# brunohs1993/Nanokappa

Hardware: AMD Instinct MI355X
Metric: phonon-steps/sec (whole node) (higher is better)
Workload: dtype f64

## Files before the change

include/nanokappa_hip.h:

```cpp
#ifndef NANOKAPPA_HIP_H
#define NANOKAPPA_HIP_H
#include <stdint.h>

#ifdef __cplusplus
extern "C" {
#endif

typedef struct nk_ctx nk_ctx;

enum nk_status {
    NK_OK = 0,
    NK_ERR_HIP = -1,
    NK_ERR_ARG = -2,
    NK_ERR_CAPACITY = -3,
    NK_ERR_COMM = -4,
    NK_ERR_NODEVICE = -5
};

typedef struct {
    int32_t Q, J, NT;
    const double *omega;
    const double *group_vel;
    const double *T_grid;
    const double *lifetime;
// ... 103 lines not shown
    double place_gbps;
    double place_worst_gbps;
    int64_t box_store;
} nk_timing;

int nk_device_count(void);
int nk_mesh_crossings(int device, int64_t n_rays, const double *origins, const double *dirs, int64_t n_faces, const double *v0,
                      const double *e1, const double *e2, int skip_self, int32_t *counts);
int nk_create(nk_ctx **out, int device_id, uint64_t seed);
void nk_destroy(nk_ctx *ctx);
const char *nk_last_error(const nk_ctx *ctx);

int nk_set_material(nk_ctx *ctx, const nk_material *m);
int nk_set_mesh(nk_ctx *ctx, const nk_mesh *m);
int nk_set_subvolumes(nk_ctx *ctx, const nk_subvols *s, const double *T_sv_init );
int nk_set_reservoirs(nk_ctx *ctx, const nk_reservoirs *r);
int nk_set_rough(nk_ctx *ctx, const nk_rough *r);
int nk_set_params(nk_ctx *ctx, const nk_params *p);

int nk_reserve(nk_ctx *ctx, int64_t capacity);
int nk_upload_particles(nk_ctx *ctx, int64_t N, const double *x, const double *y, const double *z,
                        const int32_t *mode, const double *occ, const double *n_ts, const int32_t *facet,
                        const uint64_t *pid, uint64_t pid_offset);
int nk_init_boundaries(nk_ctx *ctx);
int nk_init_particles(nk_ctx *ctx, int64_t N, int64_t capacity, uint64_t pid_lo, const int32_t *unique_modes, int64_t n_unique,
                      const int64_t *sv_first);
int nk_tally_state(nk_ctx *ctx, double *E_raw, double *N_sv, double *flux_raw);
int nk_step(nk_ctx *ctx, int32_t nsteps, nk_tally *out);
int nk_download_particles(nk_ctx *ctx, int64_t capacity, double *x, double *y, double *z, int32_t *mode,
                          double *occ, double *n_ts, int32_t *facet, uint64_t *pid, int64_t *N_out);
int nk_get_subvol_temperature(nk_ctx *ctx, double *T_sv );
int nk_set_subvol_temperature(nk_ctx *ctx, const double *T_sv );
int nk_get_step(nk_ctx *ctx, int64_t *step);
int nk_get_timing(nk_ctx *ctx, nk_timing *t);

int nk_comm_unique_id(void *id128 );
int nk_comm_init(nk_ctx *ctx, const void *id128, int rank, int nranks);
typedef struct {
    int32_t rank, nranks;
    int32_t comm_rank, comm_nranks;
    int32_t device;
    int32_t selftest_ok;
    double selftest_sum;
    char pci_bus_id[32];
} nk_comm_report;
int nk_comm_info(nk_ctx *ctx, nk_comm_report *out);
int nk_comm_allreduce(nk_ctx *ctx, double *inout, int64_t n);

int nk_set_bands(nk_ctx *ctx, int32_t nbands, const int32_t *band_of_mode);
int nk_get_band_rows(nk_ctx *ctx, double *F, double *N, int64_t *steps, int32_t cap, int32_t *nrows);
int nk_tally_bands_state(nk_ctx *ctx, double *F, double *N);

typedef struct {
    double lo[3], h[3];
    int32_t n[3];
    int32_t every;
    int32_t flags;
    int64_t capacity;
} nk_field;
#define NK_FIELD_GLOBAL 1
#define NK_FIELD_TEST_SMALL_BOUND 2
int nk_set_field(nk_ctx *ctx, const nk_field *f);
int nk_get_field(nk_ctx *ctx, double *N, double *E, double *F, int64_t *samples, int64_t *clamped, int32_t reset);
int nk_tally_field_state(nk_ctx *ctx, int64_t *raw, int64_t *clamped);
typedef struct {
    int32_t n[3], every;
// ... 84 lines not shown
```

nanokappa_amd/csrc/nk_device.h:

```cpp
#pragma once
#include <hip/hip_runtime.h>
#include <stdint.h>

#define NK_WG 256
#ifndef NK_NREP
#define NK_NREP 8
#endif
#define NK_PLANE_DOUBLES 6
#define NK_FACE_DOUBLES 16
#define NK_LDS_FACES 256
#define NK_LDS_RESFACES 64
#define NK_TAU_ROWS 3
#define NK_MAX_SEGMENTS 16384
#define NK_EMIT_CHUNK 128
#define NK_LREC 128
#define NK_NEWBORN 0x80000000u
#define NK_LOST 0x40000000u

#define NK_TAG_REFLECT 0x00000u
#define NK_TAG_EMIT 0x10000u
#define NK_TAG_RESAMP 0x20000u
#define NK_TAG_DICE 0x30000u
#define NK_TAG_INIT 0x40000u

// ... 42 lines not shown
    const int32_t *m2s;
    const int32_t *s2m;
    const int32_t *seg_nl;
    int32_t tau_row0;
    double tau_g[NK_TAU_ROWS];
    double tau_ig[NK_TAU_ROWS - 1];
    double T0, invT0;
    double c_hk;
    const double *tau;
    const double *Tgrid;
    int32_t nE;
    const double *Tarr, *Earr;
    double Tfill_lo, Tfill_hi;
    double hbar, kb, QV;
    double active_modes;
    int32_t F, Fc, NP;
    const float *tree_boxes;
    double tree_bound;
    const int32_t *tree_tags;
    const double *facet_skip;
    const double *tree_faces;
    int32_t tree_base[8];
    int32_t tree_top, tree_leaves;
    int32_t tree_nfam, tree_lds_fam0, tree_lds_off;
    int32_t NG;
    const double *planes;
    const double *faces;
    const NkFacet *facets;
    double tol;
    double bbox[6];
    int32_t box;
    double box_k[6];
    uint64_t box_ids;
    double inv_dt;
    const double *face_verts;
    const int32_t *facet_face_off;
    const int32_t *facet_face_idx;
    const double *facet_face_cdf;
    int32_t nS;
    const double *simplex_pts;
    const double *simplex_cdf;
    int32_t S, sv_kind, sv_axis, sv_interp;
    const double *centers;
    const double *sv_volume;
    double sv_lo, sv_invL;
    double *T_sv;
    const double *rbf_inv;
    int32_t rbf_P, rbf_used[3];
    double rbf_shift[3], rbf_scale[3];
    int32_t R, res_gen;
    const int32_t *res_facet;
    const double *res_T;
    const int32_t *res_face_off;
    const double *res_face_cdf;
    const double *res_face_verts;
    int32_t res_nf;
    int32_t res_lds;
    const double *enter_prob;
    double *res_counter;
    const double *ep_p;
    double *rc_p;
    int64_t rc_len;
    const double *res_roulette;
    int32_t *nleave_prev;
    uint64_t *sp_inbox;
    int32_t *sp_inbox_n;
// ... 359 lines not shown
    NkHit h = {__builtin_inf(), 0x7fffffff, -1};
    {
#pragma clang fp contract(off)
        const double2 *P = reinterpret_cast<const double2 *>(planes);
        double tmin = __builtin_inf();
        int pmin = -1, ties = 0;
        double2 n0 = P[0], n1 = P[1];
        for (int pl = 0; pl < NP; ++pl) {
            const double2 p01 = n0, p23 = n1;
            if (pl + 1 < NP) { n0 = P[3 * pl + 3]; n1 = P[3 * pl + 4]; }
            const double num = x * p01.x + y * p01.y + z * p23.x + p23.y;
            const double den = vx * p01.x + vy * p01.y + vz * p23.x;
            if (!((num < 0.0 && den > 0.0) || (num > 0.0 && den < 0.0))) continue;
            const double t = -num / den;
            if (!(t >= tol) || isinf(t)) continue;
            if (t < tmin) { tmin = t; pmin = pl; ties = 0; }
            else if (t == tmin) ties = 1;
        }
        if (pmin < 0) { tc = h.t; fc = h.facet; return; }
        if (!ties) {
            const double cx = x + tmin * vx, cy = y + tmin * vy, cz = z + tmin * vz;
            const double pr = planes[NK_PLANE_DOUBLES * pmin + 4];
            nk_fb_faces(faces, __double2loint(pr), __double2hiint(pr), tol, tmin, cx, cy, cz, h);
            if (h.facet >= 0 || h.face != 0x7fffffff) { tc = h.t; fc = h.facet; return; }
        }
    }
    nk_fb_planes(planes, faces, 0, NP, tol, x, y, z, vx, vy, vz, h);
    tc = h.t;
    fc = h.facet;
}
struct NkBoxWalls {
    double lx, hx, ly, hy, lz, hz;
    uint32_t ids_lo, ids_hi;
    __device__ __forceinline__ void load(const NkDev &d) {
        lx = d.box_k[0]; hx = -d.box_k[1]; ly = d.box_k[2]; hy = -d.box_k[3]; lz = d.box_k[4]; hz = -d.box_k[5];
        ids_lo = (uint32_t)d.box_ids; ids_hi = (uint32_t)(d.box_ids >> 32);
        asm volatile("" : "+v"(lx), "+v"(hx), "+v"(ly), "+v"(hy), "+v"(lz), "+v"(hz), "+v"(ids_lo), "+v"(ids_hi));
    }
};
__device__ __forceinline__ bool nk_box_out(const NkBoxWalls &b, double x, double y, double z, double vx, double vy, double vz) {
    const bool ox = ((x > b.hx) & (vx > 0.0)) | ((x < b.lx) & (vx < 0.0));
    const bool oy = ((y > b.hy) & (vy > 0.0)) | ((y < b.ly) & (vy < 0.0));
    const bool oz = ((z > b.hz) & (vz > 0.0)) | ((z < b.lz) & (vz < 0.0));
    return ox | oy | oz;
}
__device__ __forceinline__ void nk_box_axis(double xa, double va, double lo, double hi, int wlo, uint64_t ids,
                                            double &nb, double &db, int &wb) {
#pragma clang fp contract(off)
    const bool fwd = va > 0.0;
    const double num = fwd ? xa - hi : lo - xa;
    const double den = fabs(va);
    const int w = wlo + (fwd ? 1 : 0);
    const double l = num * db, r = nb * den;
    const unsigned f0w = (unsigned)(ids >> (8 * w + 4)) & 15u, f0b = wb < 0 ? 16u : ((unsigned)(ids >> (8 * wb + 4)) & 15u);
    if ((num > 0.0) & (den > 0.0) & ((l > r) | ((l == r) & (f0w < f0b)))) { nb = num; db = den; wb = w; }
}
__device__ __forceinline__ void nk_box_first_hit(const NkBoxWalls &b, double inv_dt, double x, double y, double z, double vx, double vy,
                                                 double vz, double &nts, int &facet) {
    const uint64_t ids = ((uint64_t)b.ids_hi << 32) | b.ids_lo;
    double nb = -1.0, db = 1.0;
    int wb = -1;
    nk_box_axis(x, vx, b.lx, b.hx, 0, ids, nb, db, wb);
    nk_box_axis(y, vy, b.ly, b.hy, 2, ids, nb, db, wb);
    nk_box_axis(z, vz, b.lz, b.hz, 4, ids, nb, db, wb);
    nts = -(nb * nk_rcp(db)) * inv_dt;
    facet = wb < 0 ? -1 : (int)((ids >> (8 * wb)) & 15u);
}
__device__ __forceinline__ void nk_box_next_axis(double xa, double va, double lo, double hi, int wlo, uint64_t ids, double tol,
                                                 double &mb, double &db, int &wb) {
#pragma clang fp contract(off)
    const bool fwd = va > 0.0;
    const double num = fwd ? xa - hi : lo - xa;
    const double den = fabs(va), m = -num;
    const int w = wlo + (fwd ? 1 : 0);
    const double l = m * db, r = mb * den;
    const unsigned f0w = (unsigned)(ids >> (8 * w + 4)) & 15u, f0b = wb < 0 ? 16u : ((unsigned)(ids >> (8 * wb + 4)) & 15u);
    if ((num < 0.0) & (den > 0.0) & (m >= tol * den) & ((wb < 0) | (l < r) | ((l == r) & (f0w < f0b)))) { mb = m; db = den; wb = w; }
// ... 217 lines not shown
#endif
        const double r = r_diff * rlast;
        int flat;
        if (hi - lo <= 4) {
            const double a0 = lo + 0 < hi ? roul[lo + 0] : __builtin_inf(), a1 = lo + 1 < hi ? roul[lo + 1] : __builtin_inf(),
                         a2 = lo + 2 < hi ? roul[lo + 2] : __builtin_inf(), a3 = lo + 3 < hi ? roul[lo + 3] : __builtin_inf();
            flat = lo + (a0 < r ? 1 : 0) + (a1 < r ? 1 : 0) + (a2 < r ? 1 : 0) + (a3 < r ? 1 : 0);
            if (flat > hi) flat = hi;
        } else flat = lo + nk_ss_left(roul + lo, hi - lo, r);
        if (flat > d.M - 1) flat = d.M - 1;
        mode_out = flat;
        omega_out = d.modetab[flat].omega;
        E0_out = d.modetab[flat].E0;
        double invT;
        nk_interp_T<RBF>(d, tb, cx, cy, cz, invT);
        n_out = nk_be(omega_out * d.c_hk, E0_out, invT, d.invT0);
    }
}

struct NkBins {
    double *E, *flux, *resb;
    unsigned int *N, *nleave, *misc;
};

struct NkParticle {
    double x, y, z, occ, nts, omega, E0, vx, vy, vz;
    int mode, facet;
    int slot;
};

#define NK_EV_DONE 0
#define NK_EV_DEAD 1
#define NK_EV_MORE 2
template <bool ROUGH, bool RBF = true>
__device__ __forceinline__ int nk_event_pre(const NkDev &d, const NkFacet *facets, const NkSvTab &tb, const double *resT, NkBins &b,
                                            NkParticle &p, double &cts, uint32_t ev, uint64_t pid, uint32_t step) {
    const double dt = d.dt;
    int fi = p.facet < 0 ? d.Fc - 1 : p.facet;
    const NkFacet fc = facets[fi];
    if (fc.bc == 'T' || fc.bc == 'F') {
        int r = p.facet < 0 ? -1 : fc.res;
        if (r >= 0) {
            const double n0 = d.T_ref_local ? nk_be(p.omega * d.c_hk, p.E0, resT[2 * r + 1], d.invT0)
                                            : nk_occupation(d, d.T_ref, p.omega, p.E0);
            double e = d.hbar * p.omega * (p.occ - n0);
            const double evn = e * nk_rcp(p.vx * fc.nx + p.vy * fc.ny + p.vz * fc.nz);
            atomicAdd(&b.nleave[r], 1u);
            atomicAdd(&b.resb[4 * r + 0], -e);
            atomicAdd(&b.resb[4 * r + 1], evn * p.vx);
            atomicAdd(&b.resb[4 * r + 2], evn * p.vy);
            atomicAdd(&b.resb[4 * r + 3], evn * p.vz);
        }
        return NK_EV_DEAD;
    }
    double tcol = p.nts * dt;
    double cx = p.x + p.vx * tcol, cy = p.y + p.vy * tcol, cz = p.z + p.vz * tcol;
    cts += (cts == 0.0) ? fabs(p.nts + 1.0) : fabs(p.nts);
    if (fc.bc == 'P') {
        p.x = cx + fc.tx; p.y = cy + fc.ty; p.z = cz + fc.tz;
    } else if (ROUGH) {
        double r0, r1;
        nk_uniform2_dev(d.seed, pid, step, NK_TAG_REFLECT + ev, r0, r1);
        p.x = cx; p.y = cy; p.z = cz;
        int mo; double no, oo, eo;
        nk_reflect<RBF>(d, tb, fc.rough, p.mode, cx, cy, cz, p.occ, p.omega, p.E0, r0, r1, r1, mo, no, oo, eo);
        p.mode = mo; p.occ = no; p.omega = oo; p.E0 = eo;
        const NkMode *rec = d.modetab + mo;
        if (d.part) p.slot = d.m2s[mo];
        p.vx = rec->vx; p.vy = rec->vy; p.vz = rec->vz;
    }
    return NK_EV_MORE;
}
__device__ __forceinline__ int nk_event_post(const NkDev &d, NkParticle &p, double &cts, uint32_t &ev, double tc, int fcn) {
    const double dt = d.dt;
    p.nts = tc / dt;
    p.facet = fcn;
    if (++ev > 4096u) cts = 1.0;
    if (cts < 1.0) {
        const double rem = 1.0 - cts;
        if (rem > p.nts) return NK_EV_MORE;
        p.x += p.vx * dt * rem; p.y += p.vy * dt * rem; p.z += p.vz * dt * rem;
        p.nts -= rem;
    }
    return NK_EV_DONE;
}
// ... 32 lines not shown
```

nanokappa_amd/csrc/nk_engine.hip:

```cpp
#include <hip/hip_runtime.h>
#include <dlfcn.h>
#include <math.h>
#include <stdio.h>
#include <stdlib.h>
#include <string.h>
#include <algorithm>
#include <functional>
#include <queue>
#include <string>
#include <type_traits>
#include <chrono>
#include <time.h>
#include <vector>

#include <rccl/rccl.h>

#include "../../include/nanokappa_hip.h"
#include "nk_kernels.h"
#include "nk_field.h"
#include "nk_modes.h"
#include "nk_group.h"
#ifndef NK_PLAIN_IN_ENGINE
extern template __global__ void k_sweep<1, false, false, false, false, true, 1>(NkDev, uint32_t, int, int);
extern template __global__ void k_sweep<1, false, false, false, false, true, 2>(NkDev, uint32_t, int, int);
extern template __global__ void k_sweep<1, false, false, false, false, false, 1>(NkDev, uint32_t, int, int);
extern template __global__ void k_sweep<1, false, false, false, false, false, 2>(NkDev, uint32_t, int, int);
extern template __global__ void k_sweep<1, false, false, false, false, true, 1, true>(NkDev, uint32_t, int, int);
extern template __global__ void k_sweep<1, false, false, false, false, true, 2, true>(NkDev, uint32_t, int, int);
extern template __global__ void k_sweep<1, false, false, false, false, false, 1, true>(NkDev, uint32_t, int, int);
extern template __global__ void k_sweep<1, false, false, false, false, false, 2, true>(NkDev, uint32_t, int, int);
#endif

struct NkRccl {
    void *lib = nullptr;
    ncclResult_t (*GetUniqueId)(ncclUniqueId *) = nullptr;
    ncclResult_t (*CommInitRank)(ncclComm_t *, int, ncclUniqueId, int) = nullptr;
    ncclResult_t (*AllReduce)(const void *, void *, size_t, ncclDataType_t, ncclRedOp_t, ncclComm_t, hipStream_t) = nullptr;
    ncclResult_t (*CommDestroy)(ncclComm_t) = nullptr;
    ncclResult_t (*CommCount)(const ncclComm_t, int *) = nullptr;
    ncclResult_t (*CommUserRank)(const ncclComm_t, int *) = nullptr;
    ncclResult_t (*CommAbort)(ncclComm_t) = nullptr;
};

static thread_local std::string g_create_error;

struct nk_ctx {
    int device = 0;
    hipStream_t stream = nullptr;
    std::string err;
    NkDev d;
    std::vector<void *> allocs;
    std::vector<void *> pallocs;
    void *store_buf = nullptr;
    size_t store_pad = 0;
    bool store_pid = false;
    bool store_nts = true;
    bool mesh_box = false;
    bool box_forbidden = false;
    int32_t *anomalies = nullptr;
    bool have_material = false, have_mesh = false, have_sv = false, have_params = false;
    int64_t step = 0;
    bool pending_relax = false;
    int g_sweep = 0;
    std::vector<int32_t> h_seg_count;
    std::vector<hipEvent_t> evpool;
    int g_sweep_key = -1;
    size_t g_sweep_lds = 0;
    int layout_key = -1;
    std::vector<double> h_enter_prob;
    int64_t spec_M = 0;
    double *spec_v = nullptr, *spec_om = nullptr, *spec_dl = nullptr, *spec_svx = nullptr;
    int32_t *spec_rank = nullptr;
    double spec_vmax = 0.0;
    NkSpecMode *spec_modes = nullptr;
    int32_t *spec_in = nullptr, *spec_out = nullptr;
    unsigned long long *spec_count = nullptr;
    double *ks_kv = nullptr, *ks_mat = nullptr;
    double ks_tol[3] = {0, 0, 0};
    int64_t ks_Q = 0;
    int64_t spec_cap = 0;
    int64_t spec_last = 0;
    int rb_Fr = 0;
    double *rb_k2 = nullptr, *rb_nin = nullptr, *rb_eta = nullptr, *rb_sub = nullptr, *rb_spec = nullptr, *rb_roul = nullptr;
    uint8_t *rb_ts = nullptr;
    unsigned int *rb_map = nullptr;
    std::vector<int32_t> rb_facet;
    int64_t o2o_first = 0;
    bool stepped = false;
    int64_t emitted_for = -1;
    std::vector<double> h_vg;
// ... 703 lines not shown
            if (seen & (1 << w)) { ok = false; break; }
            seen |= 1 << w;
            const double wall = sgn ? -pn[3] : pn[3];
            if (!(fabs(wall - m->bbox[(sgn ? 3 : 0) + a]) <= 1e-9 * (1.0 + fabs(wall)))) { ok = false; break; }
            if (members[pl].size() != 2) { ok = false; break; }
            int fct0 = -1, face0 = 0x7fffffff;
            double area = 0.0;
            for (int f : members[pl]) {
                if (fct0 < 0) fct0 = m->face_facet[f]; else if (m->face_facet[f] != fct0) ok = false;
                face0 = std::min(face0, f);
                area += m->face_area[f];
                const double *V = m->vertices + 9 * (size_t)f;
                for (int c = 0; c < 3 && ok; ++c)
                    for (int k = 0; k < 3; ++k) {
                        const double v = V[3 * c + k], lo = m->bbox[k], hi = m->bbox[3 + k];
                        const double e = 1e-9 * (1.0 + fabs(lo) + fabs(hi));
                        if (k == a) { if (fabs(v - wall) > e) ok = false; }
                        else if (fabs(v - lo) > e && fabs(v - hi) > e) ok = false;
                    }
            }
            const int b = (a + 1) % 3, c = (a + 2) % 3;
            const double side = (m->bbox[3 + b] - m->bbox[b]) * (m->bbox[3 + c] - m->bbox[c]);
            if (!(fabs(area - side) <= 1e-9 * side) || fct0 < 0 || fct0 >= m->Fc) ok = false;
            if (!ok) break;
            d.box_k[w] = pn[3];
            box_facet[w] = fct0;
            d.box_ids = (d.box_ids & ~(0xFFull << (8 * w))) | ((uint64_t)(fct0 & 15) << (8 * w)) | ((uint64_t)(face0 & 15) << (8 * w + 4));
        }
        if (ok && seen == 63) {
            int fm = 0;
            for (int w = 0; w < 6; ++w) fm |= 1 << box_facet[w];
            ctx->mesh_box = fm == 63;
        }
    }
    ctx->have_mesh = true;
    return NK_OK;
}

static inline bool nk_want_box(const nk_ctx *ctx) {
    return ctx->have_mesh && ctx->mesh_box && !ctx->box_forbidden && !getenv("NK_NO_BOX") && !getenv("NK_SPLIT") && !nk_layout_soa() &&
           ctx->d.F <= NK_LDS_FACES && ctx->d.Fc <= NK_LDS_FACES;
}

static int nk_patch_facets(nk_ctx *ctx) {
    NK_HIP(hipMemcpy((void *)ctx->d.facets, ctx->host_facets.data(), (size_t)ctx->d.Fc * sizeof(NkFacet), hipMemcpyHostToDevice));
    return NK_OK;
}

static int nk_entry_tables_drop(nk_ctx *ctx, bool keep_counters) {
    NkDev &d = ctx->d;
    if (ctx->rm_nseg > 0 && keep_counters && d.R > 0 && d.res_counter) {
        const int64_t n = (int64_t)d.R * d.M;
        k_perm_rm<<<(int)((n + 255) / 256), 256, 0, ctx->stream>>>(0, d.R, d.M, ctx->rm_nseg, ctx->rm_nlmax,
                                                                   d.m2s, d.res_counter, ctx->rc_p + (ctx->step & 1) * d.rc_len);
        NK_HIP(hipGetLastError());
        NK_HIP(hipStreamSynchronize(ctx->stream));
    }
    if (ctx->ep_p) { hipFree(ctx->ep_p); ctx->ep_p = nullptr; }
    if (ctx->rc_p) { hipFree(ctx->rc_p); ctx->rc_p = nullptr; }
    d.ep_p = nullptr; d.rc_p = nullptr;
    ctx->rm_nseg = 0;
    return NK_OK;
}
static int nk_entry_tables_build(nk_ctx *ctx) {
    NkDev &d = ctx->d;
    if (!(d.R > 0 && d.nseg > 0 && d.m2s && d.enter_prob && d.res_counter) || ctx->rm_nseg == d.nseg) return NK_OK;
    int rc = nk_entry_tables_drop(ctx, true);
    if (rc) return rc;
    const size_t len = (size_t)d.nseg * d.R * d.nlmax;
    NK_HIP(hipMalloc((void **)&ctx->ep_p, len * 8));
    NK_HIP(hipMalloc((void **)&ctx->rc_p, 2 * len * 8));
    NK_HIP(hipMemsetAsync(ctx->ep_p, 0, len * 8, ctx->stream));
    NK_HIP(hipMemsetAsync(ctx->rc_p, 0, 2 * len * 8, ctx->stream));
    d.rc_len = (int64_t)len;
// ... 535 lines not shown
    } else best = 0;
    for (size_t k = 1; k < cand.size(); ++k) hipFree(cand[k]);
    const double gb = 2.0 * (double)d.nseg * tiles * 64 * (pbytes - (ctx->store_pid ? 8 : 0)) / 1e9;
    ctx->timing.place_tries = (int64_t)cand.size();
    ctx->timing.place_gbps = ms[best] > 0.0 ? gb / (ms[best] * 1e-3) : 0.0;
    ctx->timing.place_worst_gbps = ms[worst] > 0.0 ? gb / (ms[worst] * 1e-3) : 0.0;
    if (rc) {
        if (getenv("NK_VERBOSE")) fprintf(stderr, "[nanokappa_hip] store placement: probe failed (%s); the store stays where it is\n", ctx->err.c_str());
        (void)hipGetLastError();
        rc = NK_OK;
    }
    if (getenv("NK_VERBOSE")) {
        fprintf(stderr, "[nanokappa_hip] store placement: %zu allocation(s) of %.0f MB probed:", cand.size(), (double)bytes / 1048576.0);
        for (size_t k = 0; k < ms.size(); ++k) fprintf(stderr, " %.1f", ms[k] * 1e3);
        fprintf(stderr, " us per pass; kept number %zu (%.2f TB/s); %.1f ms\n", best, ctx->timing.place_gbps / 1e3,
                std::chrono::duration<double, std::milli>(std::chrono::steady_clock::now() - wall0).count());
    }
    return rc;
}

static inline int64_t nk_tiled_count(int64_t u, int64_t nu, int64_t pid_lo, int64_t N) {
    const int64_t first = pid_lo % nu;
    return N / nu + (((u - first + nu) % nu) < N % nu ? 1 : 0);
}
static int nk_alloc_particles(nk_ctx *ctx, int64_t capacity, const int32_t *mode = nullptr, int64_t N = 0,
                              const int32_t *umodes = nullptr, int64_t nu = 0, int64_t pid_lo = 0) {
    if (ctx) ctx->emitted_for = -1;
    NkDev &d = ctx->d;
    { int rc0 = nk_entry_tables_drop(ctx, true); if (rc0) return rc0; }
    for (void *p : ctx->pallocs) hipFree(p);
    ctx->pallocs.clear();
    d.part = nk_want_part(ctx) ? 1 : 0;
    d.box = nk_want_box(ctx) ? 1 : 0;
    d.nlrec = 0;
    int64_t nseg = 0;
    for (int round = 0; round < 4; ++round) {
        const int64_t waves = (int64_t)nk_sweep_blocks(ctx) * (NK_WG / 64);
        int64_t ns = capacity / 128;
        if (const char *e = getenv("NK_SEGMENTS")) ns = atoi(e) > 0 ? atoi(e) : ns;
        else if (ns >= waves) ns = waves;
        ns = ns < 64 ? 64 : (ns > NK_MAX_SEGMENTS ? NK_MAX_SEGMENTS : ns);
        const bool same = ns == nseg;
        nseg = ns;
        d.nseg = (int32_t)nseg;
        d.nlmax = d.M > 0 ? (int32_t)((d.M + nseg - 1) / nseg) : 1;
        if (d.part && d.M > nseg) d.nlmax += d.nlmax / 6 + 2;
        d.nlrec = 0;
        if (d.part && d.nlmax <= NK_LREC && !getenv("NK_NO_LREC")) {
            const int without = nk_sweep_blocks(ctx);
            d.nlrec = d.nlmax;
            if (nk_sweep_blocks(ctx) < without) d.nlrec = 0;
        }
        if (same) break;
    }
    NK_ARG(d.nlmax < (1 << 14), "too many modes per segment for k_emit's packed entry word: use more particles (segments) or fewer modes");
    { int rcm = nk_build_mode_map(ctx); if (rcm) return rcm; }
    {
        const int64_t maxidx = d.part ? d.nlmax - 1 : (d.M > 0 ? d.M - 1 : 0);
        int lb = 1;
        while ((1ll << lb) <= maxidx) ++lb;
        NK_ARG(lb < 30 && (int64_t)d.Fc + 1 < (1ll << (31 - lb)), "mesh has too many facets for the packed particle word (facets x modes)");
        d.lb = lb;
    }
    int64_t segcap = (capacity + nseg - 1) / nseg;
    if (d.part && (mode || umodes) && N > 0) {
        std::vector<int64_t> per((size_t)nseg, 0);
// ... 1292 lines not shown
    if (x) memcpy(x, h.x.data(), live * 8);
    if (y) memcpy(y, h.y.data(), live * 8);
    if (z) memcpy(z, h.z.data(), live * 8);
    if (occ) memcpy(occ, h.occ.data(), live * 8);
    if (n_ts) memcpy(n_ts, h.nts.data(), live * 8);
    if (mode) memcpy(mode, h.mode.data(), live * 4);
    if (facet) memcpy(facet, h.facet.data(), live * 4);
    if (pid) memcpy(pid, h.pid.data(), live * 8);
    return NK_OK;
}

int nk_get_subvol_temperature(nk_ctx *ctx, double *T_sv) {
    NK_ARG(ctx && T_sv && ctx->have_sv, "nk_get_subvol_temperature: bad arguments");
    NK_HIP(hipSetDevice(ctx->device));
    NK_HIP(hipStreamSynchronize(ctx->stream));
    NK_HIP(hipMemcpy(T_sv, ctx->d.T_sv, (size_t)ctx->d.S * 8, hipMemcpyDeviceToHost));
    return NK_OK;
}
int nk_set_subvol_temperature(nk_ctx *ctx, const double *T_sv) {
    NK_ARG(ctx && T_sv && ctx->have_sv, "nk_set_subvol_temperature: bad arguments");
    NK_HIP(hipSetDevice(ctx->device));
    NK_HIP(hipStreamSynchronize(ctx->stream));
    std::vector<double> t(T_sv, T_sv + ctx->d.S);
    if (ctx->d.sv_interp == 3) nk_rbf_coefficients(ctx, t);
    NK_HIP(hipMemcpy(ctx->d.T_sv, t.data(), t.size() * 8, hipMemcpyHostToDevice));
    nk_track_T(ctx, T_sv, ctx->d.S);
    return NK_OK;
}
int nk_get_step(nk_ctx *ctx, int64_t *step) {
    NK_ARG(ctx && step, "nk_get_step: NULL argument");
    *step = ctx->step;
    return NK_OK;
}
int nk_get_timing(nk_ctx *ctx, nk_timing *t) {
    NK_ARG(ctx && t, "nk_get_timing: NULL argument");
    *t = ctx->timing;
    t->box_store = (ctx->d.cap > 0 && ctx->d.box) ? 1 : 0;
    return NK_OK;
}

static int nk_load_rccl(NkRccl &r, std::string &err) {
    if (r.lib) return NK_OK;
    const char *names[] = {"librccl.so.1", "librccl.so", "/opt/rocm/lib/librccl.so.1", "/opt/rocm/lib/librccl.so"};
    for (const char *n : names) { r.lib = dlopen(n, RTLD_NOW | RTLD_GLOBAL); if (r.lib) break; }
    if (!r.lib) { err = std::string("cannot load librccl: ") + dlerror(); return NK_ERR_COMM; }
    r.GetUniqueId = (decltype(r.GetUniqueId))dlsym(r.lib, "ncclGetUniqueId");
    r.CommInitRank = (decltype(r.CommInitRank))dlsym(r.lib, "ncclCommInitRank");
    r.AllReduce = (decltype(r.AllReduce))dlsym(r.lib, "ncclAllReduce");
    r.CommDestroy = (decltype(r.CommDestroy))dlsym(r.lib, "ncclCommDestroy");
    r.CommCount = (decltype(r.CommCount))dlsym(r.lib, "ncclCommCount");
    r.CommUserRank = (decltype(r.CommUserRank))dlsym(r.lib, "ncclCommUserRank");
    r.CommAbort = (decltype(r.CommAbort))dlsym(r.lib, "ncclCommAbort");
    if (!r.GetUniqueId || !r.CommInitRank || !r.AllReduce || !r.CommDestroy || !r.CommCount || !r.CommUserRank) { err = "librccl lacks expected symbols"; return NK_ERR_COMM; }
    return NK_OK;
}
int nk_comm_unique_id(void *id128) {
    static NkRccl r;
    std::string err;
    if (!id128) return NK_ERR_ARG;
    if (nk_load_rccl(r, err)) { g_create_error = err; return NK_ERR_COMM; }
    ncclUniqueId id;
    memset(&id, 0, sizeof(id));
    if (r.GetUniqueId(&id) != ncclSuccess) { g_create_error = "ncclGetUniqueId failed"; return NK_ERR_COMM; }
    memcpy(id128, &id, 128);
    return NK_OK;
}
// ... 799 lines not shown
```

nanokappa_amd/csrc/nk_kernels.h:

```cpp
#pragma once
#ifndef NK_KERNEL_LINKAGE
#define NK_KERNEL_LINKAGE
#endif
#include "nk_device.h"

#define NK_TILE 64
#ifndef NK_NT
#define NK_NT 0
#endif
#if NK_NT
#define NK_LD(p) __builtin_nontemporal_load(p)
#define NK_ST(p, v) __builtin_nontemporal_store(v, p)
#else
#define NK_LD(p) (*(p))
#define NK_ST(p, v) (*(p) = (v))
#endif
#ifdef NK_STAMPS
#define NK_STAMP(k)                                                                                    \
    do {                                                                                               \
        unsigned long long t_;                                                                         \
        __builtin_amdgcn_sched_barrier(0);                                                             \
        asm volatile("s_memtime %0\n\ts_waitcnt lgkmcnt(0)" : "=s"(t_)::"memory");                     \
        __builtin_amdgcn_sched_barrier(0);                                                             \
        st_acc[k] += t_ - st_last;                                                                     \
// ... 729 lines not shown
                    }
                }
                sev = false;
            }
            if (PF2) fetch(buf, (t + 2) * NK_TILE);
            if (!flush) {
                const int r = t * NK_TILE;
                if (!PF2) fetch(buf, r + NK_TILE);
                const bool newborn = (w0 & NK_NEWBORN) != 0u;
                w0 &= ~NK_NEWBORN;
                const int idx = act ? (int)(w0 & lbmask) : 0;
                double4 ra, rb;
                if (use_lrec) {
                    const NkLdsRec q = nk_lds_rec(lrec + idx * NK_LREC_STRIDE);
                    const nk_v2d q0 = q[0], q1 = q[1], q2 = q[2], q3 = q[3];
                    ra = make_double4(q0.x, q0.y, q1.x, q1.y); rb = make_double4(q2.x, q2.y, q3.x, q3.y);
                }
                else { const double4 *g = reinterpret_cast<const double4 *>(sm.rec + idx); ra = g[0]; rb = g[1]; }
                omega = ra.x; vx = ra.y; vy = ra.z; vz = ra.w; E0 = rb.x;
#ifdef NK_STAMPS
                { const double fence_ = x + omega; asm volatile("" ::"v"(fence_)); }
#endif
                NK_STAMP(0);
                if (act && !newborn) {
                    if (do_relax) occ = nk_relax<RBF>(d, L, tw, ra, rb, x, y, z, occ, sm, idx);
                    x += vx * d.dt; y += vy * d.dt; z += vz * d.dt;
                    if (!BOX) nts -= 1.0;
                }
#ifdef NK_STAMPS
                { const double fence_ = x + occ; asm volatile("" ::"v"(fence_)); }
#endif
                NK_STAMP(1);
            }
            const bool ev = BOX ? (act && (w0 & NK_LOST) == 0u && nk_box_out(bw, x, y, z, vx, vy, vz)) : (act && nts < 0.0);
            const bool done = act && !ev;
            const unsigned long long mD = __ballot(done), mE = __ballot(ev);
            if (done) nk_tally_one(d, L.tb, L.bins, x, y, z, occ, omega, E0, vx, vy, vz, do_flux, rep);
            if (DEFER) {
                so = O.reserve(nk_rank(mD), __popcll(mD));
                sdone = done; sx = x; sy = y; sz = z; socc = occ; snts = nts; sw0 = w0; spid = pid;
            } else O.template push<BOX>(d, base, lane, done, nk_rank(mD), __popcll(mD), x, y, z, occ, nts, w0, pid);
            NK_STAMP(2);
            if (SPLIT) {
                if (DEFER) { sev = ev; sq = qn + nk_rank(mE); }
                else if (ev) {
                    const int o = qn + nk_rank(mE);
                    if (o < d.segcap) {
                        const int64_t i = base + o;
                        d.qx[i] = x; d.qy[i] = y; d.qz[i] = z; d.qocc[i] = occ; d.qnts[i] = nts; d.qw0[i] = w0;
                        if (PID) d.qpid[i] = pid;
                    }
                }
                qn += __popcll(mE);
                return;
            }
            const int pn = __popcll(mE), erank = nk_rank(mE);
            int taken = 0;
            while (taken < pn || (flush && cn > 0)) {
                if (taken < pn) {
                    const int k = pn - taken < 64 - cn ? pn - taken : 64 - cn;
                    if (ev && erank >= taken && erank < taken + k) {
                        const int sl = cn + erank - taken;
                        cX[sl] = x; cX[64 + sl] = y; cX[128 + sl] = z; cX[192 + sl] = occ; cX[256 + sl] = nts; cX[320 + sl] = 0.0;
                        cW[sl] = w0; cW[64 + sl] = 0u;
                        if (PID) { cP[sl] = __longlong_as_double((long long)pid); cW[128 + sl] = (uint32_t)mode_of((int)(w0 & lbmask)); cW[192 + sl] = (w0 & lbmask) * (uint32_t)d.nseg + (uint32_t)seg; }
                    }
                    cn += k; taken += k;
                }
// ... 1616 lines not shown
```

nanokappa_amd/engine.py:

```python
import ctypes as C
import os

import numpy as np

_HERE = os.path.dirname(os.path.abspath(__file__))
LIB_PATH = os.path.join(_HERE, os.environ.get('NK_LIBNAME', 'libnanokappa_hip.so'))

c_dp = C.POINTER(C.c_double)
c_ip = C.POINTER(C.c_int32)
c_bp = C.POINTER(C.c_int8)
c_up = C.POINTER(C.c_uint8)
c_u64p = C.POINTER(C.c_uint64)


class NkError(RuntimeError):
    pass


class nk_material(C.Structure):
    _fields_ = [('Q', C.c_int32), ('J', C.c_int32), ('NT', C.c_int32),
                ('omega', c_dp), ('group_vel', c_dp), ('T_grid', c_dp), ('lifetime', c_dp),
                ('nE', C.c_int32), ('T_fill_lo', C.c_double), ('T_fill_hi', C.c_double),
                ('T_array', c_dp), ('energy_array', c_dp),
                ('hbar', C.c_double), ('kb', C.c_double), ('QV', C.c_double), ('active_modes', C.c_int32)]
# ... 22 lines not shown
class nk_rough(C.Structure):
    _fields_ = [('Fr', C.c_int32), ('facet', c_ip), ('specularity', c_dp), ('true_spec', c_up),
                ('spec_map', c_ip), ('roulette', c_dp), ('degen_j2', c_ip)]


class nk_params(C.Structure):
    _fields_ = [('dt', C.c_double), ('norm_fixed', C.c_int32), ('particle_density', C.c_double),
                ('T_ref_local', C.c_int32), ('T_ref', C.c_double), ('flux_every', C.c_int32),
                ('contains_every', C.c_int32), ('track_ids', C.c_int32)]


class nk_tally(C.Structure):
    _fields_ = [('T_sv', c_dp), ('E_sv', c_dp), ('E_raw', c_dp), ('N_sv', c_dp), ('flux_raw', c_dp),
                ('N_leaving', c_dp), ('res_energy', c_dp), ('res_flux', c_dp), ('N_emitted', c_dp)]


class nk_timing(C.Structure):
    _fields_ = [('step_kernel_ms', C.c_double), ('emit_kernel_ms', C.c_double), ('events_kernel_ms', C.c_double),
                ('total_ms', C.c_double),
                ('slots', C.c_int64), ('live', C.c_int64),
                ('regrows', C.c_int64), ('halts', C.c_int64), ('tau_rebuilds', C.c_int64), ('batches', C.c_int64),
                ('emit_fused', C.c_int64), ('place_tries', C.c_int64), ('place_gbps', C.c_double), ('place_worst_gbps', C.c_double),
                ('box_store', C.c_int64)]


class nk_comm_report(C.Structure):
    _fields_ = [('rank', C.c_int32), ('nranks', C.c_int32), ('comm_rank', C.c_int32), ('comm_nranks', C.c_int32),
                ('device', C.c_int32), ('selftest_ok', C.c_int32), ('selftest_sum', C.c_double), ('pci_bus_id', C.c_char * 32)]


EXPORTS = ['nk_device_count', 'nk_create', 'nk_destroy', 'nk_last_error', 'nk_set_material', 'nk_set_mesh', 'nk_set_subvolumes',
           'nk_set_reservoirs', 'nk_set_rough', 'nk_set_params', 'nk_reserve', 'nk_upload_particles',
           'nk_init_boundaries', 'nk_step', 'nk_download_particles', 'nk_get_subvol_temperature',
           'nk_set_subvol_temperature', 'nk_get_step', 'nk_get_timing', 'nk_comm_unique_id', 'nk_comm_init',
           'nk_find_boundary', 'nk_classify', 'nk_eval', 'nk_reflect', 'nk_uniform2', 'nk_calibrate_stream',
           'nk_specular_begin', 'nk_specular_pairs', 'nk_specular_end', 'nk_rough_begin', 'nk_rough_pairs', 'nk_rough_finish',
           'nk_rough_download', 'nk_build_enter_prob', 'nk_init_particles', 'nk_tally_state', 'nk_kspec_begin', 'nk_kspec_pairs',
           'nk_rough_finish_k', 'nk_mesh_crossings', 'nk_comm_info', 'nk_comm_allreduce', 'nk_set_bands', 'nk_get_band_rows',
           'nk_tally_bands_state', 'nk_set_field', 'nk_get_field', 'nk_tally_field_state', 'nk_field_info',
           'nk_set_modes', 'nk_get_modes', 'nk_tally_modes_state', 'nk_modes_info',
           'nk_group_create', 'nk_group_destroy', 'nk_group_step', 'nk_group_info', 'nk_group_last_error']

class nk_field(C.Structure):
    _fields_ = [('lo', C.c_double * 3), ('h', C.c_double * 3), ('n', C.c_int32 * 3), ('every', C.c_int32), ('flags', C.c_int32),
                ('capacity', C.c_int64)]


class nk_field_report(C.Structure):
    _fields_ = [('n', C.c_int32 * 3), ('every', C.c_int32), ('ncells', C.c_int64), ('k_E', C.c_int32), ('k_F', C.c_int32),
                ('B_E', C.c_double), ('B_F', C.c_double), ('capacity', C.c_int64), ('bytes', C.c_int64),
                ('lds_path', C.c_int32), ('on', C.c_int32)]


class nk_modes(C.Structure):
    _fields_ = [('every', C.c_int32), ('flags', C.c_int32), ('capacity', C.c_int64)]


class nk_modes_report(C.Structure):
    _fields_ = [('every', C.c_int32), ('k_E', C.c_int32), ('B_E', C.c_double), ('capacity', C.c_int64), ('bytes', C.c_int64),
                ('owner_path', C.c_int32), ('on', C.c_int32)]


class nk_group_report(C.Structure):
    _fields_ = [('R', C.c_int32), ('halted', C.c_int32), ('finished_alone', C.c_int32), ('grid_sweep', C.c_int32),
                ('grid_tail', C.c_int32), ('pad_', C.c_int32), ('steps', C.c_int64), ('sweep_launches', C.c_int64),
                ('tail_launches', C.c_int64), ('member_launches', C.c_int64), ('sweep_kernel_ms', C.c_double),
                ('tail_kernel_ms', C.c_double), ('total_ms', C.c_double)]
# ... 8 lines not shown

_lib = None


def load_library():
    global _lib
    if _lib is not None:
        return _lib
    if not os.path.exists(LIB_PATH):
        raise NkError('%s not found: build it with `make -C %s` (needs hipcc); there is no CPU fallback'
                      % (LIB_PATH, os.path.join(_HERE, 'csrc')))
    L = C.CDLL(LIB_PATH)
    L.nk_last_error.restype = C.c_char_p
    L.nk_last_error.argtypes = [C.c_void_p]
    L.nk_create.argtypes = [C.POINTER(C.c_void_p), C.c_int, C.c_uint64]
    L.nk_destroy.argtypes = [C.c_void_p]
    L.nk_destroy.restype = None
    for name, st in (('nk_set_material', nk_material), ('nk_set_mesh', nk_mesh), ('nk_set_reservoirs', nk_reservoirs),
                     ('nk_set_rough', nk_rough), ('nk_set_params', nk_params)):
        getattr(L, name).argtypes = [C.c_void_p, C.POINTER(st)]
    L.nk_set_subvolumes.argtypes = [C.c_void_p, C.POINTER(nk_subvols), c_dp]
    L.nk_reserve.argtypes = [C.c_void_p, C.c_int64]
    L.nk_upload_particles.argtypes = [C.c_void_p, C.c_int64, c_dp, c_dp, c_dp, c_ip, c_dp, c_dp, c_ip, c_u64p, C.c_uint64]
    L.nk_init_boundaries.argtypes = [C.c_void_p]
    L.nk_init_particles.argtypes = [C.c_void_p, C.c_int64, C.c_int64, C.c_uint64, c_ip, C.c_int64, C.POINTER(C.c_int64)]
    L.nk_tally_state.argtypes = [C.c_void_p, c_dp, c_dp, c_dp]
    L.nk_mesh_crossings.argtypes = [C.c_int, C.c_int64, c_dp, c_dp, C.c_int64, c_dp, c_dp, c_dp, C.c_int, c_ip]
    L.nk_step.argtypes = [C.c_void_p, C.c_int32, C.POINTER(nk_tally)]
    L.nk_download_particles.argtypes = [C.c_void_p, C.c_int64, c_dp, c_dp, c_dp, c_ip, c_dp, c_dp, c_ip, c_u64p,
                                        C.POINTER(C.c_int64)]
    L.nk_get_subvol_temperature.argtypes = [C.c_void_p, c_dp]
    L.nk_set_subvol_temperature.argtypes = [C.c_void_p, c_dp]
    L.nk_get_step.argtypes = [C.c_void_p, C.POINTER(C.c_int64)]
    L.nk_get_timing.argtypes = [C.c_void_p, C.POINTER(nk_timing)]
    L.nk_comm_unique_id.argtypes = [C.c_void_p]
    L.nk_comm_init.argtypes = [C.c_void_p, C.c_void_p, C.c_int, C.c_int]
    L.nk_comm_info.argtypes = [C.c_void_p, C.POINTER(nk_comm_report)]
    L.nk_comm_allreduce.argtypes = [C.c_void_p, c_dp, C.c_int64]
    L.nk_find_boundary.argtypes = [C.c_void_p, C.c_int64, c_dp, c_dp, c_dp, c_dp, c_ip]
    L.nk_classify.argtypes = [C.c_void_p, C.c_int64, c_dp, c_ip]
    L.nk_eval.argtypes = [C.c_void_p, C.c_int32, C.c_int64, c_dp, c_ip, c_dp]
    L.nk_reflect.argtypes = [C.c_void_p, C.c_int64, c_ip, c_ip, c_dp, c_dp, c_dp, c_dp, c_dp, c_dp, c_ip, c_dp, c_dp]
    L.nk_uniform2.argtypes = [C.c_uint64, C.c_uint64, C.c_uint32, C.c_uint32, c_dp, c_dp]
    L.nk_calibrate_stream.argtypes = [C.c_void_p, C.c_int32, C.POINTER(C.c_int64), C.POINTER(C.c_int64)]
    L.nk_specular_begin.argtypes = [C.c_void_p, C.c_int64, c_dp, c_dp, c_dp]
    L.nk_specular_pairs.argtypes = [C.c_void_p, c_dp, C.c_double, C.c_int64, c_ip, c_ip, C.POINTER(C.c_int64)]
    L.nk_specular_end.argtypes = [C.c_void_p]
    L.nk_rough_begin.argtypes = [C.c_void_p, C.c_int32, c_ip, c_dp, c_dp, c_dp]
    L.nk_rough_pairs.argtypes = [C.c_void_p, C.c_int32, c_ip]
    L.nk_rough_finish.argtypes = [C.c_void_p]
    L.nk_rough_finish_k.argtypes = [C.c_void_p, C.c_int32, c_ip, c_ip]
    L.nk_kspec_begin.argtypes = [C.c_void_p, C.c_int64, c_dp, c_dp, c_dp, c_dp]
    L.nk_kspec_pairs.argtypes = [C.c_void_p, c_dp, C.c_int64, c_ip, c_ip, C.POINTER(C.c_int64)]
    L.nk_rough_download.argtypes = [C.c_void_p, c_dp, c_up, c_ip, c_dp]
    L.nk_build_enter_prob.argtypes = [C.c_void_p, C.c_int32, c_dp, c_dp, C.c_double, c_dp]
    L.nk_set_bands.argtypes = [C.c_void_p, C.c_int32, c_ip]
    L.nk_get_band_rows.argtypes = [C.c_void_p, c_dp, c_dp, C.POINTER(C.c_int64), C.c_int32, c_ip]
    L.nk_tally_bands_state.argtypes = [C.c_void_p, c_dp, c_dp]
    c_i64p = C.POINTER(C.c_int64)
    L.nk_set_field.argtypes = [C.c_void_p, C.POINTER(nk_field)]
    L.nk_get_field.argtypes = [C.c_void_p, c_dp, c_dp, c_dp, c_i64p, c_i64p, C.c_int32]
    L.nk_tally_field_state.argtypes = [C.c_void_p, c_i64p, c_i64p]
    L.nk_field_info.argtypes = [C.c_void_p, C.POINTER(nk_field_report)]
    L.nk_set_modes.argtypes = [C.c_void_p, C.POINTER(nk_modes)]
    L.nk_get_modes.argtypes = [C.c_void_p, c_dp, c_dp, c_i64p, c_i64p, C.c_int32]
    L.nk_tally_modes_state.argtypes = [C.c_void_p, c_i64p, c_i64p]
# ... 334 lines not shown
        kE = self.modes_info()['k_E']
        return dict(N_raw=N, E_raw=E, k_E=kE, N=N.astype(np.float64), E=np.ldexp(E.astype(np.float64), -kE))

    def get_step(self):
        n = C.c_int64(0)
        self._ck(self.L.nk_get_step(self.h, C.byref(n)), 'nk_get_step')
        return int(n.value)

    def download(self):
        n = C.c_int64(0)
        self._ck(self.L.nk_download_particles(self.h, 0, None, None, None, None, None, None, None, None, C.byref(n)),
                 'nk_download_particles')
        N = int(n.value)
        x, y, z, occ, nts = (np.zeros(N) for _ in range(5))
        mode, facet = np.zeros(N, dtype=np.int32), np.zeros(N, dtype=np.int32)
        pid = np.zeros(N, dtype=np.uint64)
        if N:
            self._ck(self.L.nk_download_particles(self.h, N, _p(x), _p(y), _p(z), _p(mode, c_ip), _p(occ), _p(nts),
                                                  _p(facet, c_ip), _p(pid, c_u64p), C.byref(n)), 'nk_download_particles')
        return dict(positions=np.stack((x, y, z), axis=1), mode=mode, occupation=occ, n_timesteps=nts, facet=facet, pid=pid)

    def subvol_temperature(self):
        t = np.zeros(self.S)
        self._ck(self.L.nk_get_subvol_temperature(self.h, _p(t)), 'nk_get_subvol_temperature')
        return t

    def set_subvol_temperature(self, T):
        t = _d(T)
        self._ck(self.L.nk_set_subvol_temperature(self.h, _p(t)), 'nk_set_subvol_temperature')

    def timing(self):
        t = nk_timing()
        self._ck(self.L.nk_get_timing(self.h, C.byref(t)), 'nk_get_timing')
        return dict(step_kernel_ms=t.step_kernel_ms, emit_kernel_ms=t.emit_kernel_ms, events_kernel_ms=t.events_kernel_ms,
                    total_ms=t.total_ms,
                    slots=int(t.slots), live=int(t.live), regrows=int(t.regrows), halts=int(t.halts),
                    tau_rebuilds=int(t.tau_rebuilds), batches=int(t.batches), emit_fused=int(t.emit_fused),
                    place_tries=int(t.place_tries), place_gbps=t.place_gbps, place_worst_gbps=t.place_worst_gbps,
                    box_store=int(t.box_store))

    def specular_begin(self, group_vel, omega, delta_omega):
        v, om, dl = _d(np.asarray(group_vel).reshape(-1, 3)), _d(np.ravel(omega)), _d(np.ravel(delta_omega))
        self._ck(self.L.nk_specular_begin(self.h, om.shape[0], _p(v), _p(om), _p(dl)), 'nk_specular_begin')
        self._spec_M = om.shape[0]

    def specular_pairs(self, normal, crit=1e-3, download=True):
        nrm = _d(np.asarray(normal, dtype=float))
        cap = getattr(self, '_spec_cap', 4 * self._spec_M)
        while True:
            n = C.c_int64(0)
            if download:
                pi, po = np.empty(cap, dtype=np.int32), np.empty(cap, dtype=np.int32)
                self._ck(self.L.nk_specular_pairs(self.h, _p(nrm), float(crit), cap, _p(pi, c_ip), _p(po, c_ip), C.byref(n)),
                         'nk_specular_pairs')
            else:
                self._ck(self.L.nk_specular_pairs(self.h, _p(nrm), float(crit), cap, None, None, C.byref(n)), 'nk_specular_pairs')
            if n.value <= cap:
                return (pi[:n.value].astype(np.int64), po[:n.value].astype(np.int64)) if download else None
            cap = self._spec_cap = int(n.value)

    def specular_end(self):
        self._ck(self.L.nk_specular_end(self.h), 'nk_specular_end')

    def rough_begin(self, facets, normal_in, eta, k_norm):
        f, n, e, k = _i(facets), _d(normal_in), _d(eta), _d(k_norm)
        self._rough_Fr = f.shape[0]
        self._ck(self.L.nk_rough_begin(self.h, f.shape[0], _p(f, c_ip), _p(n), _p(e), _p(k)), 'nk_rough_begin')

    def rough_pairs(self, rough_facet_indices):
        f = _i(rough_facet_indices)
        self._ck(self.L.nk_rough_pairs(self.h, f.shape[0], _p(f, c_ip)), 'nk_rough_pairs')

# ... 147 lines not shown
```

Baseline: 53.42 billion.

## Resolve periodic wraps and reservoir absorption inline in box-mesh step kernel

```diff
diff --git a/include/nanokappa_hip.h b/include/nanokappa_hip.h
--- a/include/nanokappa_hip.h
+++ b/include/nanokappa_hip.h
@@ -159,6 +159,7 @@
 int nk_get_subvol_temperature(nk_ctx *ctx, double *T_sv );
 int nk_set_subvol_temperature(nk_ctx *ctx, const double *T_sv );
 int nk_get_step(nk_ctx *ctx, int64_t *step);
+int nk_get_box_inline(nk_ctx *ctx, int64_t *mask);
 int nk_get_timing(nk_ctx *ctx, nk_timing *t);
 
 int nk_comm_unique_id(void *id128 );
diff --git a/nanokappa_amd/csrc/nk_device.h b/nanokappa_amd/csrc/nk_device.h
--- a/nanokappa_amd/csrc/nk_device.h
+++ b/nanokappa_amd/csrc/nk_device.h
@@ -98,6 +98,8 @@
     int32_t box;
     double box_k[6];
     uint64_t box_ids;
+    uint32_t box_inline;
+    double box_wrap[3];
     double inv_dt;
     const double *face_verts;
     const int32_t *facet_face_off;
@@ -523,10 +525,15 @@
 struct NkBoxWalls {
     double lx, hx, ly, hy, lz, hz;
     uint32_t ids_lo, ids_hi;
+    double wx, wy, wz;
+    uint32_t inl;
     __device__ __forceinline__ void load(const NkDev &d) {
         lx = d.box_k[0]; hx = -d.box_k[1]; ly = d.box_k[2]; hy = -d.box_k[3]; lz = d.box_k[4]; hz = -d.box_k[5];
         ids_lo = (uint32_t)d.box_ids; ids_hi = (uint32_t)(d.box_ids >> 32);
+        wx = d.box_wrap[0]; wy = d.box_wrap[1]; wz = d.box_wrap[2];
+        inl = d.box_inline;
         asm volatile("" : "+v"(lx), "+v"(hx), "+v"(ly), "+v"(hy), "+v"(lz), "+v"(hz), "+v"(ids_lo), "+v"(ids_hi));
+        asm volatile("" : "+v"(wx), "+v"(wy), "+v"(wz), "+v"(inl));
     }
 };
 __device__ __forceinline__ bool nk_box_out(const NkBoxWalls &b, double x, double y, double z, double vx, double vy, double vz) {
@@ -534,6 +541,11 @@
     const bool oy = ((y > b.hy) & (vy > 0.0)) | ((y < b.ly) & (vy < 0.0));
     const bool oz = ((z > b.hz) & (vz > 0.0)) | ((z < b.lz) & (vz < 0.0));
     return ox | oy | oz;
+}
+__device__ __forceinline__ uint32_t nk_box_beyond(const NkBoxWalls &b, double x, double y, double z, double vx, double vy, double vz) {
+    return (((x < b.lx) & (vx < 0.0)) ? 1u : 0u) | (((x > b.hx) & (vx > 0.0)) ? 2u : 0u) |
+           (((y < b.ly) & (vy < 0.0)) ? 4u : 0u) | (((y > b.hy) & (vy > 0.0)) ? 8u : 0u) |
+           (((z < b.lz) & (vz < 0.0)) ? 16u : 0u) | (((z > b.hz) & (vz > 0.0)) ? 32u : 0u);
 }
 __device__ __forceinline__ void nk_box_axis(double xa, double va, double lo, double hi, int wlo, uint64_t ids,
                                             double &nb, double &db, int &wb) {
@@ -817,6 +829,18 @@
 #define NK_EV_DONE 0
 #define NK_EV_DEAD 1
 #define NK_EV_MORE 2
+__device__ __forceinline__ void nk_absorb_tally(const NkDev &d, const double *resT, NkBins &b, int r, double nx, double ny, double nz,
+                                                double occ, double omega, double E0, double vx, double vy, double vz) {
+    const double n0 = d.T_ref_local ? nk_be(omega * d.c_hk, E0, resT[2 * r + 1], d.invT0)
+                                    : nk_occupation(d, d.T_ref, omega, E0);
+    double e = d.hbar * omega * (occ - n0);
+    const double evn = e * nk_rcp(vx * nx + vy * ny + vz * nz);
+    atomicAdd(&b.nleave[r], 1u);
+    atomicAdd(&b.resb[4 * r + 0], -e);
+    atomicAdd(&b.resb[4 * r + 1], evn * vx);
+    atomicAdd(&b.resb[4 * r + 2], evn * vy);
+    atomicAdd(&b.resb[4 * r + 3], evn * vz);
+}
 template <bool ROUGH, bool RBF = true>
 __device__ __forceinline__ int nk_event_pre(const NkDev &d, const NkFacet *facets, const NkSvTab &tb, const double *resT, NkBins &b,
                                             NkParticle &p, double &cts, uint32_t ev, uint64_t pid, uint32_t step) {
@@ -825,17 +849,7 @@
     const NkFacet fc = facets[fi];
     if (fc.bc == 'T' || fc.bc == 'F') {
         int r = p.facet < 0 ? -1 : fc.res;
-        if (r >= 0) {
-            const double n0 = d.T_ref_local ? nk_be(p.omega * d.c_hk, p.E0, resT[2 * r + 1], d.invT0)
-                                            : nk_occupation(d, d.T_ref, p.omega, p.E0);
-            double e = d.hbar * p.omega * (p.occ - n0);
-            const double evn = e * nk_rcp(p.vx * fc.nx + p.vy * fc.ny + p.vz * fc.nz);
-            atomicAdd(&b.nleave[r], 1u);
-            atomicAdd(&b.resb[4 * r + 0], -e);
-            atomicAdd(&b.resb[4 * r + 1], evn * p.vx);
-            atomicAdd(&b.resb[4 * r + 2], evn * p.vy);
-            atomicAdd(&b.resb[4 * r + 3], evn * p.vz);
-        }
+        if (r >= 0) nk_absorb_tally(d, resT, b, r, fc.nx, fc.ny, fc.nz, p.occ, p.omega, p.E0, p.vx, p.vy, p.vz);
         return NK_EV_DEAD;
     }
     double tcol = p.nts * dt;
diff --git a/nanokappa_amd/csrc/nk_engine.hip b/nanokappa_amd/csrc/nk_engine.hip
--- a/nanokappa_amd/csrc/nk_engine.hip
+++ b/nanokappa_amd/csrc/nk_engine.hip
@@ -56,6 +56,7 @@
     bool store_pid = false;
     bool store_nts = true;
     bool mesh_box = false;
+    uint32_t mesh_box_inline = 0;
     bool box_forbidden = false;
     int32_t *anomalies = nullptr;
     bool have_material = false, have_mesh = false, have_sv = false, have_params = false;
@@ -825,6 +826,27 @@
             for (int w = 0; w < 6; ++w) fm |= 1 << box_facet[w];
             ctx->mesh_box = fm == 63;
         }
+        ctx->mesh_box_inline = 0;
+        if (ctx->mesh_box) {
+            const std::vector<NkFacet> &hf = ctx->host_facets;
+            bool rough = false;
+            for (int w = 0; w < 6; ++w) rough = rough || hf[(size_t)box_facet[w]].bc == 'R';
+            for (int a = 0; a < 3; ++a) {
+                const NkFacet &lo = hf[(size_t)box_facet[2 * a]], &hi = hf[(size_t)box_facet[2 * a + 1]];
+                const double tl[3] = {lo.tx, lo.ty, lo.tz}, th[3] = {hi.tx, hi.ty, hi.tz};
+                const int b = (a + 1) % 3, c = (a + 2) % 3;
+                d.box_wrap[a] = 0.0;
+                if (lo.bc == 'P' && hi.bc == 'P' && lo.partner == box_facet[2 * a + 1] && hi.partner == box_facet[2 * a] &&
+                    tl[b] == 0.0 && tl[c] == 0.0 && th[b] == 0.0 && th[c] == 0.0 && tl[a] > 0.0 && th[a] == -tl[a]) {
+                    ctx->mesh_box_inline |= 3u << (2 * a);
+                    d.box_wrap[a] = tl[a];
+                }
+                for (int s = 0; s < 2; ++s) {
+                    const int bc = hf[(size_t)box_facet[2 * a + s]].bc;
+                    if ((bc == 'T' || bc == 'F') && !rough) ctx->mesh_box_inline |= 1u << (8 + 2 * a + s);
+                }
+            }
+        }
     }
     ctx->have_mesh = true;
     return NK_OK;
@@ -833,6 +855,11 @@
 static inline bool nk_want_box(const nk_ctx *ctx) {
     return ctx->have_mesh && ctx->mesh_box && !ctx->box_forbidden && !getenv("NK_NO_BOX") && !getenv("NK_SPLIT") && !nk_layout_soa() &&
            ctx->d.F <= NK_LDS_FACES && ctx->d.Fc <= NK_LDS_FACES;
+}
+
+static inline uint32_t nk_box_inline(const nk_ctx *ctx) {
+    if (!nk_want_box(ctx) || getenv("NK_NO_BOX_INLINE")) return 0u;
+    return getenv("NK_NO_BOX_ABSORB") ? (ctx->mesh_box_inline & 63u) : ctx->mesh_box_inline;
 }
 
 static int nk_patch_facets(nk_ctx *ctx) {
@@ -1434,6 +1461,7 @@
     ctx->pallocs.clear();
     d.part = nk_want_part(ctx) ? 1 : 0;
     d.box = nk_want_box(ctx) ? 1 : 0;
+    d.box_inline = nk_box_inline(ctx);
     d.nlrec = 0;
     int64_t nseg = 0;
     for (int round = 0; round < 4; ++round) {
@@ -2792,6 +2820,11 @@
     *step = ctx->step;
     return NK_OK;
 }
+int nk_get_box_inline(nk_ctx *ctx, int64_t *mask) {
+    NK_ARG(ctx && mask, "nk_get_box_inline: NULL argument");
+    *mask = (ctx->d.cap > 0 && ctx->d.box) ? (int64_t)ctx->d.box_inline : 0;
+    return NK_OK;
+}
 int nk_get_timing(nk_ctx *ctx, nk_timing *t) {
     NK_ARG(ctx && t, "nk_get_timing: NULL argument");
     *t = ctx->timing;
diff --git a/nanokappa_amd/csrc/nk_kernels.h b/nanokappa_amd/csrc/nk_kernels.h
--- a/nanokappa_amd/csrc/nk_kernels.h
+++ b/nanokappa_amd/csrc/nk_kernels.h
@@ -785,8 +785,35 @@
 #endif
                 NK_STAMP(1);
             }
-            const bool ev = BOX ? (act && (w0 & NK_LOST) == 0u && nk_box_out(bw, x, y, z, vx, vy, vz)) : (act && nts < 0.0);
-            const bool done = act && !ev;
+            bool ev, gone = false;
+            if (BOX) {
+                const bool live = act && (w0 & NK_LOST) == 0u;
+                const uint32_t inl = (uint32_t)__builtin_amdgcn_readfirstlane((int)bw.inl);
+                {
+                    const uint32_t pm = inl & 63u, am = (inl >> 8) & 63u;
+                    const uint32_t mv = live ? nk_box_beyond(bw, x, y, z, vx, vy, vz) : 0u;
+                    ev = mv != 0u;
+                    if (pm != 0u) {
+                        double nx = x, ny = y, nz = z;
+                        if (pm & 3u) nx = (mv & 3u) ? x + ((mv & 1u) ? bw.wx : -bw.wx) : x;
+                        if (pm & 12u) ny = (mv & 12u) ? y + ((mv & 4u) ? bw.wy : -bw.wy) : y;
+                        if (pm & 48u) nz = (mv & 48u) ? z + ((mv & 16u) ? bw.wz : -bw.wz) : z;
+                        if (ev && (mv & ~pm) == 0u && !nk_box_out(bw, nx, ny, nz, vx, vy, vz)) { x = nx; y = ny; z = nz; ev = false; }
+                    }
+                    if (am != 0u) {
+                        const uint32_t A = mv & am;
+                        if (A != 0u && (A & (A - 1u)) == 0u && (mv & ~(pm | am)) == 0u) {
+                            const int wa = __builtin_ctz(A);
+                            const uint64_t ids = ((uint64_t)bw.ids_hi << 32) | bw.ids_lo;
+                            const NkFacet &fc = L.facets[(int)((ids >> (8 * wa)) & 15u)];
+                            const int r = fc.res;
+                            if (r >= 0) nk_absorb_tally(d, L.resT, L.bins, r, fc.nx, fc.ny, fc.nz, occ, omega, E0, vx, vy, vz);
+                            ev = false; gone = true;
+                        }
+                    }
+                }
+            } else ev = act && nts < 0.0;
+            const bool done = act && !ev && !gone;
             const unsigned long long mD = __ballot(done), mE = __ballot(ev);
             if (done) nk_tally_one(d, L.tb, L.bins, x, y, z, occ, omega, E0, vx, vy, vz, do_flux, rep);
             if (DEFER) {
diff --git a/nanokappa_amd/engine.py b/nanokappa_amd/engine.py
--- a/nanokappa_amd/engine.py
+++ b/nanokappa_amd/engine.py
@@ -78,7 +78,7 @@
 EXPORTS = ['nk_device_count', 'nk_create', 'nk_destroy', 'nk_last_error', 'nk_set_material', 'nk_set_mesh', 'nk_set_subvolumes',
            'nk_set_reservoirs', 'nk_set_rough', 'nk_set_params', 'nk_reserve', 'nk_upload_particles',
            'nk_init_boundaries', 'nk_step', 'nk_download_particles', 'nk_get_subvol_temperature',
-           'nk_set_subvol_temperature', 'nk_get_step', 'nk_get_timing', 'nk_comm_unique_id', 'nk_comm_init',
+           'nk_set_subvol_temperature', 'nk_get_step', 'nk_get_box_inline', 'nk_get_timing', 'nk_comm_unique_id', 'nk_comm_init',
            'nk_find_boundary', 'nk_classify', 'nk_eval', 'nk_reflect', 'nk_uniform2', 'nk_calibrate_stream',
            'nk_specular_begin', 'nk_specular_pairs', 'nk_specular_end', 'nk_rough_begin', 'nk_rough_pairs', 'nk_rough_finish',
            'nk_rough_download', 'nk_build_enter_prob', 'nk_init_particles', 'nk_tally_state', 'nk_kspec_begin', 'nk_kspec_pairs',
@@ -153,6 +153,7 @@
     L.nk_get_subvol_temperature.argtypes = [C.c_void_p, c_dp]
     L.nk_set_subvol_temperature.argtypes = [C.c_void_p, c_dp]
     L.nk_get_step.argtypes = [C.c_void_p, C.POINTER(C.c_int64)]
+    L.nk_get_box_inline.argtypes = [C.c_void_p, C.POINTER(C.c_int64)]
     L.nk_get_timing.argtypes = [C.c_void_p, C.POINTER(nk_timing)]
     L.nk_comm_unique_id.argtypes = [C.c_void_p]
     L.nk_comm_init.argtypes = [C.c_void_p, C.c_void_p, C.c_int, C.c_int]
@@ -553,12 +554,14 @@
     def timing(self):
         t = nk_timing()
         self._ck(self.L.nk_get_timing(self.h, C.byref(t)), 'nk_get_timing')
+        m = C.c_int64(0)
+        self._ck(self.L.nk_get_box_inline(self.h, C.byref(m)), 'nk_get_box_inline')
         return dict(step_kernel_ms=t.step_kernel_ms, emit_kernel_ms=t.emit_kernel_ms, events_kernel_ms=t.events_kernel_ms,
                     total_ms=t.total_ms,
                     slots=int(t.slots), live=int(t.live), regrows=int(t.regrows), halts=int(t.halts),
                     tau_rebuilds=int(t.tau_rebuilds), batches=int(t.batches), emit_fused=int(t.emit_fused),
                     place_tries=int(t.place_tries), place_gbps=t.place_gbps, place_worst_gbps=t.place_worst_gbps,
-                    box_store=int(t.box_store))
+                    box_store=int(t.box_store), box_inline=int(m.value))
 
     def specular_begin(self, group_vel, omega, delta_omega):
         v, om, dl = _d(np.asarray(group_vel).reshape(-1, 3)), _d(np.ravel(omega)), _d(np.ravel(delta_omega))
```

Result: slower. 51.75 billion (-3.1%).
